# Intsights/PySubstringSearch

Hardware: AMD Instinct MI355X
Metric: queries/sec (batched) + index-build GB/s on 512MB chunk, 1/2/4/8 GPU (higher is better)
Workload: dtype u64

## Files before the change

pysubstringsearch_amd/csrc/msd_sort.hip:

```cpp
#include "msd_sort.h"

#include <algorithm>
#include <vector>

#include "prims.h"
#include "scan.h"
#include "text_keys.h"

namespace pss {

constexpr int MSD_D = 10;
constexpr u32 MSD_BINS = 1u << MSD_D;
constexpr int MSD_BLOCK = 512;
constexpr int MSD_WAVES = MSD_BLOCK / kWave;
constexpr int MSD_IPT = 16;
constexpr u32 MSD_TILE = MSD_BLOCK * MSD_IPT;
constexpr u32 MSD_WIN = 6144;
#ifndef PSS_LS_WINDOW
#define PSS_LS_WINDOW 8
#endif
constexpr u32 MSD_TILE_CAP = 8184 - PSS_LS_WINDOW;
constexpr u32 MSD_MAX_BUCKET = 4088;
constexpr int MSD_TAG_BITS = MSD_D + 1;
constexpr u32 MSD_TAG_SPAN = 1u << MSD_TAG_BITS;
// ... 682 lines not shown
struct InNonEmpty {
    const u32 *J;
    __device__ u64 operator()(u64 j) const { return J[j + 1] > J[j] ? 1u : 0u; }
};

__global__ __launch_bounds__(256) void msd_compact_kernel(const u32 *J, u32 nb, const u64 *rank, u32 *cstart, u32 *counters, u32 *cj)
{
    u32 mx = 0;
    for (u32 j = blockIdx.x * blockDim.x + threadIdx.x; j < nb; j += gridDim.x * blockDim.x) {
        const u32 s = J[j], e = J[j + 1];
        if (e > s) {
            cstart[rank[j]] = s;
            if (cj) cj[rank[j]] = j;
            mx = max(mx, e - s);
        }
    }
    mx = wave_incl_max(mx);
    if (lane_id() == kWave - 1 && mx) atomicMax(&counters[1], mx);
}

struct TilePlan {
    u32 win, cap;
    const u32 *cj;
};
__device__ __forceinline__ bool msd_tile_head(const u32 *cstart, u32 ne, u32 n, u32 k, TilePlan tp)
{
    if (tp.cj) {
        if (k == 0 || (tp.cj[k] >> MSD_RAW_TAG_BITS) != (tp.cj[k - 1] >> MSD_RAW_TAG_BITS)) return true;
    } else if ((k & (MSD_TAG_SPAN - 1u)) == 0) {
        return true;
    }
    const u32 w = cstart[k] / tp.win;
    if (cstart[k - 1] / tp.win != w) return true;
    if (k + 1 < ne && cstart[k + 1] / tp.win == w) return false;
    u32 lo = 0, hi = k;
    const u32 ws = w * tp.win;
    while (lo < hi) {
        const u32 mid = (lo + hi) >> 1;
        if (cstart[mid] < ws) lo = mid + 1; else hi = mid;
    }
    const u32 end = k + 1 < ne ? cstart[k + 1] : n;
    return end - cstart[lo] > tp.cap;
}

struct InTileHead {
    const u32 *cstart;
    u32 ne, n;
    TilePlan tp;
    __device__ u64 operator()(u64 k) const { return msd_tile_head(cstart, ne, n, (u32)k, tp) ? 1u : 0u; }
};

struct InTileHeadDev {
    const u32 *cstart;
    const u64 *nep;
    u32 n;
    TilePlan tp;
    __device__ u64 operator()(u64 k) const
    {
        const u32 ne = (u32)*nep;
        return (k < ne && msd_tile_head(cstart, ne, n, (u32)k, tp)) ? 1u : 0u;
    }
};
__global__ __launch_bounds__(256) void msd_tiles_dev_kernel(const u32 *cstart, const u64 *nep, u32 n, const u64 *rank, const u64 *total,
                                                              u32 *tile_first, TilePlan tp)
{
    const u32 ne = (u32)*nep;
    if (blockIdx.x == 0 && threadIdx.x == 0) tile_first[*total] = ne;
    for (u32 k = blockIdx.x * blockDim.x + threadIdx.x; k < ne; k += gridDim.x * blockDim.x) {
        if (msd_tile_head(cstart, ne, n, k, tp)) tile_first[rank[k]] = k;
    }
}

__global__ __launch_bounds__(256) void msd_tiles_kernel(const u32 *cstart, u32 ne, u32 n, const u64 *rank, const u64 *total,
                                                          u32 *tile_first, TilePlan tp)
{
    if (blockIdx.x == 0 && threadIdx.x == 0) tile_first[*total] = ne;
    for (u32 k = blockIdx.x * blockDim.x + threadIdx.x; k < ne; k += gridDim.x * blockDim.x) {
        if (msd_tile_head(cstart, ne, n, k, tp)) tile_first[rank[k]] = k;
    }
}

struct MsdTile {
    u32 e0, count, tag0, nb;
};


struct MsdEmit {
    u32 *st_pos, *st_idx;
    u32 *blk_cnt;
};

__device__ __forceinline__ void msd_emit_tile(const u64 *exch, u32 count, u32 e0, int idx_bits, u32 *sa_out, const MsdEmit *em,
                                              u32 *s_count)
{
    const u32 tid = threadIdx.x, lane = tid & 63u;
    const u32 imask = (u32)((1ull << idx_bits) - 1ull);
    const u32 rows = (count + MSD_BLOCK - 1) / MSD_BLOCK;
#pragma unroll 1
    for (u32 r = 0; r < rows; ++r) {
        const u32 p = r * MSD_BLOCK + tid;
        const bool valid = p < count;
        u64 x = 0;
        bool tie = false;
        if (valid) {
            x = exch[p];
            tie = p > 0 && (exch[p - 1] >> idx_bits) == (x >> idx_bits);
            sa_out[e0 + p] = ((u32)x & imask) | ((tie && em == nullptr) ? 0x80000000u : 0u);
        }
        if (em != nullptr) {
            const u64 tm = __ballot(tie);
            const bool tie_next = lane < 63 ? ((tm >> (lane + 1)) & 1ull) != 0
                                            : (p + 1 < count && (exch[p + 1] >> idx_bits) == (x >> idx_bits));
            if (valid && (tie || tie_next)) {
                const u32 slot = e0 + atomicAdd(s_count, 1u);
                em->st_pos[slot] = e0 + p;
                em->st_idx[slot] = ((u32)x & imask) | (tie ? 0x80000000u : 0u);
            }
        }
    }
}

struct InBlkCnt {
    const u32 *c;
    __device__ u64 operator()(u64 t) const { return c[t]; }
};

constexpr u32 GA_WORDS = MSD_TILE / 32;
__global__ __launch_bounds__(256) void msd_gather_kernel(const MsdTile *tiles, const u32 *blk_cnt, const u64 *dst_off, u32 nt,
                                                           const u32 *st_pos, const u32 *st_idx, u32 *pos, u32 *idx, u32 *grp)
{
    __shared__ u32 s_occ[4][GA_WORDS], s_head[4][GA_WORDS], s_pre[4][GA_WORDS];
    const u32 w = wave_id(), lane = lane_id();
    const u32 t = blockIdx.x * 4 + w;
    if (t >= nt) return;
    const u32 c = blk_cnt[t];
    if (c == 0) return;
    const u32 e0 = tiles[t].e0;
    const u64 d = dst_off[t];
    u32 *occ = s_occ[w], *head = s_head[w], *pre = s_pre[w];
    for (u32 i = lane; i < GA_WORDS; i += kWave) occ[i] = head[i] = 0;
    __builtin_amdgcn_fence(__ATOMIC_ACQ_REL, "wavefront");
    __builtin_amdgcn_wave_barrier();
    for (u32 i = lane; i < c; i += kWave) {
        const u32 q = st_pos[e0 + i] - e0;
        atomicOr(&occ[q >> 5], 1u << (q & 31u));
        if (!(st_idx[e0 + i] >> 31)) atomicOr(&head[q >> 5], 1u << (q & 31u));
    }
    __builtin_amdgcn_fence(__ATOMIC_ACQ_REL, "wavefront");
    __builtin_amdgcn_wave_barrier();
    {
        const u32 c0 = __popc(occ[4 * lane]), c1 = __popc(occ[4 * lane + 1]), c2 = __popc(occ[4 * lane + 2]),
                  c3 = __popc(occ[4 * lane + 3]);
        const u32 ex = wave_incl_sum(c0 + c1 + c2 + c3) - (c0 + c1 + c2 + c3);
        pre[4 * lane] = ex;
        pre[4 * lane + 1] = ex + c0;
        pre[4 * lane + 2] = ex + c0 + c1;
        pre[4 * lane + 3] = ex + c0 + c1 + c2;
    }
    __builtin_amdgcn_fence(__ATOMIC_ACQ_REL, "wavefront");
    __builtin_amdgcn_wave_barrier();
    for (u32 i = lane; i < c; i += kWave) {
        const u32 ps = st_pos[e0 + i], q = ps - e0;
        const u32 below = (q & 31u) ? (occ[q >> 5] & ((1u << (q & 31u)) - 1u)) : 0u;
        const u32 rank = pre[q >> 5] + __popc(below);
        u32 wi = q >> 5;
        u32 m = head[wi] & ((q & 31u) == 31u ? ~0u : ((2u << (q & 31u)) - 1u));
        while (m == 0 && wi > 0) m = head[--wi];
        const u32 hq = wi * 32 + (31u - (u32)__builtin_clz(m | 1u));
        pos[d + rank] = ps;
        idx[d + rank] = st_idx[e0 + i] & 0x7fffffffu;
        grp[d + rank] = e0 + hq + 1;
    }
}


__global__ __launch_bounds__(MSD_BLOCK) void msd_local_sort_kernel(const u64 *in, const MsdTile *tiles, int rem_bits, int idx_bits,
                                                                     u32 *sa_out, const u32 *tile_list, int fused, MsdEmit em_val)
{
    const MsdEmit *em = fused ? &em_val : nullptr;
    __shared__ __attribute__((aligned(16))) u64 exch[MSD_TILE];
    __shared__ u32 wave_hist[MSD_WAVES][256];
    __shared__ u32 scr[MSD_WAVES + 1];
    const u32 tid = threadIdx.x, lane = tid & 63u, wave = tid >> 6;
    const u32 t = tile_list ? tile_list[blockIdx.x] : blockIdx.x;
    const MsdTile td = tiles[t];
    const u32 e0 = td.e0, count = td.count;
    for (u32 i = tid; i < MSD_WAVES * 256; i += MSD_BLOCK) (&wave_hist[0][0])[i] = 0;
    __syncthreads();
    int seg_bits = 0;
    while ((1u << seg_bits) < td.nb) ++seg_bits;
    const u64 tag_base = (u64)td.tag0 << (rem_bits + idx_bits);
    u64 key[MSD_IPT];
#pragma unroll
    for (int r = 0; r < MSD_IPT; ++r) {
        const u32 p = wave * (kWave * MSD_IPT) + r * kWave + lane;
        key[r] = p < count ? in[e0 + p] - tag_base : ~0ull;
    }
    const int sort_bits = rem_bits + seg_bits;
    for (int shift = idx_bits; shift < idx_bits + sort_bits; shift += 8) {
        const int left = idx_bits + sort_bits - shift;
        const u32 dmask = left >= 8 ? 0xffu : ((1u << left) - 1u);
        u32 rank[MSD_IPT], prev[MSD_IPT];
#pragma unroll
        for (int r = 0; r < MSD_IPT; ++r) {
            const bool pad = wave * (kWave * MSD_IPT) + r * kWave + lane >= count;
            const u32 d = pad ? dmask : ((u32)(key[r] >> shift) & dmask);
            const u64 peers = match_digit8(d, ~0ull);
            const u32 below = mbcnt(peers);
            prev[r] = 0;
            if (below == 0) prev[r] = atomicAdd(&wave_hist[wave][d], (u32)__popcll(peers));
            rank[r] = below | ((u32)__builtin_ctzll(peers) << 16);
        }
#pragma unroll
        for (int r = 0; r < MSD_IPT; ++r) rank[r] = __shfl(prev[r], (int)(rank[r] >> 16)) + (rank[r] & 0xffffu);
        __syncthreads();
        {
            u32 c[MSD_WAVES];
            u32 total = 0;
            if (tid < 256) {
#pragma unroll
                for (int w = 0; w < MSD_WAVES; ++w) {
                    c[w] = wave_hist[w][tid];
                    total += c[w];
                }
            }
            const u32 incl = wave_incl_sum(total);
            if (lane == kWave - 1) scr[wave] = incl;
            __syncthreads();
            if (tid < 256) {
                u32 run = incl - total;
                for (u32 w = 0; w < wave; ++w) run += scr[w];
#pragma unroll
                for (int w = 0; w < MSD_WAVES; ++w) {
                    wave_hist[w][tid] = run;
                    run += c[w];
                }
            }
        }
        __syncthreads();
#pragma unroll
        for (int r = 0; r < MSD_IPT; ++r) {
            const bool pad = wave * (kWave * MSD_IPT) + r * kWave + lane >= count;
            const u32 d = pad ? dmask : ((u32)(key[r] >> shift) & dmask);
            exch[wave_hist[wave][d] + rank[r]] = key[r];
        }
        __syncthreads();
        for (u32 i = tid; i < MSD_WAVES * 256; i += MSD_BLOCK) (&wave_hist[0][0])[i] = 0;
#pragma unroll
        for (int r = 0; r < MSD_IPT; ++r) key[r] = exch[wave * (kWave * MSD_IPT) + r * kWave + lane];
        __syncthreads();
    }
    if (sort_bits <= 0) {
#pragma unroll
        for (int r = 0; r < MSD_IPT; ++r) exch[wave * (kWave * MSD_IPT) + r * kWave + lane] = key[r];
        __syncthreads();
    }
    if (tid == 0) scr[0] = 0;
    __syncthreads();
    msd_emit_tile(exch, count, e0, idx_bits, sa_out, em, &scr[0]);
    __syncthreads();
    if (em && tid == 0) em->blk_cnt[t] = scr[0];
}


#ifndef PSS_LS_BIN_BITS
#define PSS_LS_BIN_BITS 12
#endif
constexpr int LS_BIN_BITS = PSS_LS_BIN_BITS;
constexpr u32 LS_BINS = 1u << LS_BIN_BITS;
constexpr u32 LS_WORDS = LS_BINS / 2;
constexpr u32 LS_KMAX = 64;
#ifndef PSS_LS_GROUP
#define PSS_LS_GROUP 1
#endif
constexpr int LS_GROUP = PSS_LS_GROUP;
constexpr int LS_WINDOW = PSS_LS_WINDOW;

__global__ __launch_bounds__(256) void msd_tile_desc_kernel(const u32 *cstart, const u32 *tile_first, u32 nt, u32 ne, u32 n,
                                                              MsdTile *tiles, const u32 *cj, const u64 *ntp, const u64 *nep)
{
    const u32 t = blockIdx.x * blockDim.x + threadIdx.x;
    if (ntp) {
        nt = (u32)*ntp;
        ne = (u32)*nep;
    }
    if (t >= nt) return;
    const u32 k0 = tile_first[t], k1 = tile_first[t + 1];
    const u32 e0 = cstart[k0], e1 = k1 < ne ? cstart[k1] : n;
    if (cj) {
        const u32 t0 = cj[k0] & (MSD_RAW_TAG_SPAN - 1u), t1 = cj[k1 - 1] & (MSD_RAW_TAG_SPAN - 1u);
        tiles[t] = MsdTile{e0, e1 - e0, t0, t1 - t0 + 1u};
    } else {
        tiles[t] = MsdTile{e0, e1 - e0, k0 & (MSD_TAG_SPAN - 1u), k1 - k0};
    }
}

__device__ __forceinline__ void keep_load(u64 &v) { asm volatile("" : "+v"(v)); }

__device__ __forceinline__ void lds_barrier()
{
    asm volatile("s_waitcnt lgkmcnt(0)\n\ts_barrier" ::: "memory");
}

__global__ __launch_bounds__(MSD_BLOCK, 4) void msd_local_fast_kernel(const u64 *in, const MsdTile *tiles, u32 nt, int rem_bits,
                                                                     int idx_bits, u32 *sa_out, u32 *fail_list, u32 *fail_count,
                                                                     int fused, MsdEmit em_val, const u64 *nt_dev,
                                                                     const u32 *counters_dev, const u32 *bad_dev)
{
    if (nt_dev) {
        if (counters_dev[1] > MSD_MAX_BUCKET || (bad_dev && *bad_dev)) return;
        nt = (u32)*nt_dev;
    }
    const MsdEmit *em = fused ? &em_val : nullptr;
    __shared__ __attribute__((aligned(16))) u64 lds_all[MSD_TILE + LS_WORDS];
    u64 *const exch = lds_all;
    u32 *const hist = reinterpret_cast<u32 *>(lds_all + MSD_TILE);
    u32 *const hist2 = hist + LS_WORDS;
    u32 *const scr = reinterpret_cast<u32 *>(&exch[MSD_TILE - 8]);
    u32 &s_fail = scr[MSD_WAVES + 2];
    const u32 tid = threadIdx.x;
    const u32 stride = gridDim.x;
    u32 t = blockIdx.x;
    if (t >= nt) return;
    MsdTile cur = tiles[t];
    MsdTile nxt = t + stride < nt ? tiles[t + stride] : MsdTile{0, 0, 0, 0};
    u64 pe[MSD_IPT];
    auto prefetch = [&](const MsdTile &d) {
#pragma unroll
        for (int r = 0; r < MSD_IPT; ++r) {
            const u32 p = r * MSD_BLOCK + tid;
            pe[r] = p < d.count ? in[d.e0 + p] : 0ull;
        }
    };
    prefetch(cur);
    for (u32 i = tid; i < LS_WORDS; i += MSD_BLOCK) hist[i] = 0;
    if (tid == 0) {
        s_fail = 0;
        scr[MSD_WAVES + 3] = 0;
    }
    lds_barrier();
    u32 prev_t = 0;
    bool prev_ok = false;
    for (;;) {
        const u32 count = cur.count, e0 = cur.e0;
        const u32 rows = (count + MSD_BLOCK - 1) / MSD_BLOCK;
        int seg_bits = 0;
        while ((1u << seg_bits) < cur.nb) ++seg_bits;
        const u64 tag_base = (u64)cur.tag0 << (rem_bits + idx_bits);
        const int sort_bits = rem_bits + seg_bits;
        const int bin_shift = idx_bits + (sort_bits > LS_BIN_BITS ? sort_bits - LS_BIN_BITS : 0);
        u64 e[MSD_IPT];
#pragma unroll
        for (int r = 0; r < MSD_IPT; ++r) {
            e[r] = ~0ull;
            if ((u32)r < rows) {
                const u32 p = r * MSD_BLOCK + tid;
                if (p < count) {
                    e[r] = pe[r] - tag_base;
                    const u32 bin = (u32)(e[r] >> bin_shift);
                    atomicAdd(&hist[bin >> 1], 1u << (16u * (bin & 1u)));
                }
            }
        }
        const bool more = t + stride < nt;
        if (more) prefetch(nxt);
        lds_barrier();
        if (tid == 0) {
            if (em && prev_ok) em->blk_cnt[prev_t] = scr[MSD_WAVES + 3];
            s_fail = 0;
            scr[MSD_WAVES + 3] = 0;
        }
        {
            constexpr int LS_WPT = LS_WORDS / MSD_BLOCK;
            static_assert(LS_WPT * MSD_BLOCK == (int)LS_WORDS && LS_WPT >= 1, "bins split evenly over the threads");
            u32 c[2 * LS_WPT];
            u32 sum = 0;
#pragma unroll
            for (int j = 0; j < LS_WPT; ++j) {
                const u32 wv = hist[LS_WPT * tid + j];
                c[2 * j] = wv & 0xffffu;
                c[2 * j + 1] = wv >> 16;
                sum += c[2 * j] + c[2 * j + 1];
            }
            const u32 incl = wave_incl_sum(sum);
            if (lane_id() == kWave - 1) scr[wave_id()] = incl;
            lds_barrier();
            u32 ex = incl - sum;
            for (int w = 0; w < wave_id(); ++w) ex += scr[w];
#pragma unroll
            for (int j = 0; j < LS_WPT; ++j) {
                const u32 lo = ex, hi = ex + c[2 * j];
                hist[LS_WPT * tid + j] = hist2[LS_WPT * tid + j] = lo | (hi << 16);
                ex = hi + c[2 * j + 1];
            }
        }
        lds_barrier();
#pragma unroll
        for (int r = 0; r < MSD_IPT; ++r) {
            if ((u32)r < rows) {
                const u32 p = r * MSD_BLOCK + tid;
                if (p < count) {
                    const u32 bin = (u32)(e[r] >> bin_shift), sh = 16u * (bin & 1u);
                    exch[(atomicAdd(&hist2[bin >> 1], 1u << sh) >> sh) & 0xffffu] = e[r];
                }
            }
        }
        if (tid < (u32)LS_WINDOW) exch[count + tid] = ~0ull;
        lds_barrier();
        const u16 *const starts16 = reinterpret_cast<const u16 *>(hist);
        u32 rk[MSD_IPT];
#pragma unroll
        for (int g = 0; g < MSD_IPT; g += LS_GROUP) {
            if ((u32)g < rows) {
                u64 x[LS_GROUP];
                u32 s0[LS_GROUP], sm[LS_GROUP];
#pragma unroll
                for (int j = 0; j < LS_GROUP; ++j) x[j] = exch[(g + j) * MSD_BLOCK + tid];
#pragma unroll
                for (int j = 0; j < LS_GROUP; ++j) {
                    const u32 bin = (u32)(x[j] >> bin_shift) & (LS_BINS - 1u);
                    s0[j] = starts16[bin];
                }
                u64 y[LS_GROUP][LS_WINDOW];
#pragma unroll
                for (int j = 0; j < LS_GROUP; ++j) {
#pragma unroll
                    for (int k = 0; k < LS_WINDOW; ++k) y[j][k] = exch[s0[j] + k];
                }
#pragma unroll
                for (int j = 0; j < LS_GROUP; ++j) {
                    u32 c = 0;
#pragma unroll
                    for (int k = 0; k < LS_WINDOW; ++k) {
                        keep_load(y[j][k]);
                        c += y[j][k] < x[j] ? 1u : 0u;
                    }
                    sm[j] = c;
                }
#pragma unroll
                for (int j = 0; j < LS_GROUP; ++j) {
                    const u32 p = (g + j) * MSD_BLOCK + tid;
                    if (p < count && ((y[j][LS_WINDOW - 1] ^ x[j]) >> bin_shift) == 0) {
                        const u32 bin = (u32)(x[j] >> bin_shift) & (LS_BINS - 1u);
                        const u32 s1 = bin + 1u < LS_BINS ? (u32)starts16[min(bin + 1u, LS_BINS - 1u)] : count;
                        const u32 len = s1 - s0[j];
                        if (len > LS_KMAX) {
                            s_fail = 1;
                        } else {
                            for (u32 q = s0[j] + LS_WINDOW; q < s0[j] + len; ++q) sm[j] += exch[q] < x[j] ? 1u : 0u;
                        }
                    }
                    e[g + j] = x[j];
                    rk[g + j] = s0[j] + sm[j];
                }
            } else {
#pragma unroll
                for (int j = 0; j < LS_GROUP; ++j) rk[g + j] = 0;
            }
        }
        lds_barrier();
        const bool failed = s_fail != 0;
        if (failed) {
            if (tid == 0) fail_list[atomicAdd(fail_count, 1u)] = t;
        } else {
#pragma unroll
            for (int r = 0; r < MSD_IPT; ++r) {
                if ((u32)r < rows) {
                    const u32 p = r * MSD_BLOCK + tid;
                    if (p < count) exch[rk[r]] = e[r];
                }
            }
        }
        for (u32 i = tid; i < LS_WORDS; i += MSD_BLOCK) hist[i] = 0;
        lds_barrier();
        if (!failed) {
            const u32 imask = (u32)((1ull << idx_bits) - 1ull);
            u32 *const s_count = &scr[MSD_WAVES + 3];
#pragma unroll
            for (int g = 0; g < MSD_IPT; g += LS_GROUP) {
                if ((u32)g < rows) {
                    u64 cur[LS_GROUP], prv[LS_GROUP], nxt[LS_GROUP];
#pragma unroll
                    for (int j = 0; j < LS_GROUP; ++j) {
                        const u32 p = (g + j) * MSD_BLOCK + tid;
                        cur[j] = exch[p];
                        prv[j] = exch[p ? p - 1 : 0];
                        nxt[j] = exch[p + 1];
                    }
#pragma unroll
                    for (int j = 0; j < LS_GROUP; ++j) {
                        keep_load(cur[j]);
                        keep_load(prv[j]);
                        keep_load(nxt[j]);
                    }
#pragma unroll
                    for (int j = 0; j < LS_GROUP; ++j) {
                        const u32 p = (g + j) * MSD_BLOCK + tid;
                        if (p < count) {
                            const u64 kx = cur[j] >> idx_bits;
                            const bool tie = p > 0 && (prv[j] >> idx_bits) == kx;
                            const u32 sfx = (u32)cur[j] & imask;
                            sa_out[e0 + p] = sfx | ((tie && em == nullptr) ? 0x80000000u : 0u);
                            if (em != nullptr) {
                                const bool tie_next = p + 1 < count && (nxt[j] >> idx_bits) == kx;
                                if (tie || tie_next) {
                                    const u32 slot = e0 + atomicAdd(s_count, 1u);
                                    em->st_pos[slot] = e0 + p;
                                    em->st_idx[slot] = sfx | (tie ? 0x80000000u : 0u);
                                }
                            }
                        }
                    }
                }
            }
        }
        prev_t = t;
        prev_ok = !failed;
        if (!more) break;
        t += stride;
        cur = nxt;
        nxt = t + stride < nt ? tiles[t + stride] : MsdTile{0, 0, 0, 0};
    }
    if (em) {
        lds_barrier();
        if (tid == 0 && prev_ok) em->blk_cnt[prev_t] = scr[MSD_WAVES + 3];
    }
}

#include "ss_sort_impl.h"


static size_t msd_max_tiles(uint32_t n)
{
    return (size_t)n / (SS_WIN / 2) + ((size_t)MSD_BINS * MSD_BINS) / MSD_RAW_TAG_SPAN + 8;
}

static size_t msd_max_tiles2(uint32_t n) { return (size_t)n / MSD_TILE2 + MSD_BINS + 8; }

static bool msd_use_lsd(uint32_t n)
{
    const char *e = knob("PSS_MSD_LSD");
    return !(e && atoi(e) == 0) && n < (1u << 30);
}

size_t msd_workspace_bytes(uint32_t n)
{
    const size_t max_ranges2 = (size_t)n / MSD_G2_RANGE + MSD_BINS + 8;
    const size_t nbk = (size_t)MSD_BINS * MSD_BINS;
    return max_ranges2 * MSD_BINS * 4
           + (MSD_BINS + 8) * 4
           + (nbk + 8) * 4
           + max_ranges2 * sizeof(MsdRange) + (MSD_BINS + 8) * 4 + 64
           + (nbk + 8) * 8
           + (nbk + 8) * 4
           + (msd_max_tiles(n) + 32) * 8
           + (msd_max_tiles(n) + 32) * 16
           + (msd_max_tiles(n) + 32) * sizeof(MsdTile)
           + (SC_MAX_BLOCKS + 8) * 8 + 8192
           + (size_t)MSD_BINS * MSD_G1_RANGES * 4 + (MSD_BINS + 8) * 4
           + msd_max_tiles2(n) * (sizeof(MsdTile2) + (size_t)MSD_BINS * 4)
           + (nbk + 8) * 4 + 4096;
}

int msd_max_key_bits(uint32_t n)
{
    int ib = 1;
    while ((1ull << ib) < (u64)n) ++ib;
    const int after2 = 64 + MSD_D - (msd_use_lsd(n) ? MSD_RAW_TAG_BITS : MSD_TAG_BITS) - ib + MSD_D;
    return std::min(after2, 64 + MSD_D - ib);
}

int msd_suffix_sort(DeviceCtx *ctx, const TextKeys *text, uint32_t n, int key_bits, uint64_t *A[2], uint32_t *sa_out,
                    void *work, uint32_t *h_small, bool profile, MsdStats *stats, bool *accepted, MsdActive *active,
                    const MsdFront *front)
{
    *accepted = false;
    hipStream_t s = ctx->stream;
    int ib = 1;
    while ((1ull << ib) < (u64)n) ++ib;
    if (key_bits < 2 * MSD_D + 1 || key_bits > msd_max_key_bits(n) || n < 2) {
        set_error("msd_suffix_sort: key of %d bits does not fit (n = %u)", key_bits, n);
        return PSS_EINVAL;
    }
    const size_t max_ranges2 = (size_t)n / MSD_G2_RANGE + MSD_BINS + 8;
    const size_t nbk = (size_t)MSD_BINS * MSD_BINS;
    u8 *w = static_cast<u8 *>(work);
    size_t o = 0;
    auto carve = [&](size_t bytes) { u8 *p = w + o; o = round_up(o + bytes, 256); return p; };
    u32 *T = reinterpret_cast<u32 *>(carve(max_ranges2 * MSD_BINS * 4));
    u32 *J1 = reinterpret_cast<u32 *>(carve((MSD_BINS + 8) * 4));
    u32 *J = reinterpret_cast<u32 *>(carve((nbk + 8) * 4));
    MsdRange *ranges2 = reinterpret_cast<MsdRange *>(carve(max_ranges2 * sizeof(MsdRange)));
    u32 *seg_first = reinterpret_cast<u32 *>(carve((MSD_BINS + 8) * 4));
    u32 *counters = reinterpret_cast<u32 *>(carve(64));
    u64 *ranks = reinterpret_cast<u64 *>(carve((nbk + 8) * 8));
    u32 *cstart = reinterpret_cast<u32 *>(carve((nbk + 8) * 4));
    const size_t max_tiles = msd_max_tiles(n);
    MsdTile *tiles_all = reinterpret_cast<MsdTile *>(carve((max_tiles + 16) * sizeof(MsdTile)));
    u32 *tile_first = reinterpret_cast<u32 *>(carve((max_tiles + 16) * 8));
    u32 *blk_cnt = reinterpret_cast<u32 *>(carve((max_tiles + 8) * 4));
    u64 *dst_off = reinterpret_cast<u64 *>(carve((max_tiles + 8) * 8));
    u64 *partial = reinterpret_cast<u64 *>(carve((SC_MAX_BLOCKS + 8) * 8));
    u64 *d_total = partial + SC_MAX_BLOCKS;
    const bool lsd = msd_use_lsd(n);
    const size_t max_tiles2 = msd_max_tiles2(n);
    u32 *T2 = nullptr, *Jb = nullptr, *status = nullptr, *cj = nullptr;
    MsdTile2 *tiles2 = nullptr;
    if (lsd) {
        T2 = reinterpret_cast<u32 *>(carve((size_t)MSD_BINS * MSD_G1_RANGES * 4));
        Jb = reinterpret_cast<u32 *>(carve((MSD_BINS + 8) * 4));
        tiles2 = reinterpret_cast<MsdTile2 *>(carve(max_tiles2 * sizeof(MsdTile2)));
        status = reinterpret_cast<u32 *>(carve(max_tiles2 * MSD_BINS * 4));
        cj = reinterpret_cast<u32 *>(carve((nbk + 8) * 4));
    }

    MsdArgs a;
    memset(&a, 0, sizeof a);
    a.codes = text->codes;
    a.code_bits = text->code_bits;
    a.key_chars = text->key_chars;
    a.plus_one = text->plus_one;
    a.key_drop = text->drop;
    a.n = n;
    a.key_bits = key_bits;
    a.idx_bits = ib;
    const u32 num_tiles = (u32)(((u64)n + MSD_TILE - 1) / MSD_TILE);
    a.tiles_per_range1 = (num_tiles + MSD_G1_RANGES - 1) / MSD_G1_RANGES;
    a.num_ranges1 = (num_tiles + a.tiles_per_range1 - 1) / a.tiles_per_range1;
    a.T = T;
    a.J1 = J1;
    a.J = J;
    a.ranges2 = ranges2;
    a.seg_first = seg_first;
    a.counters = counters;
    a.lsd = lsd ? 1 : 0;
    a.T2 = T2;
    a.Jb = Jb;
    a.tiles2 = tiles2;
    a.status = status;

    hipEvent_t ev[8] = {};
    int nev = 0;
    struct EvGuard {
        hipEvent_t *e;
        int *n;
        ~EvGuard()
        {
            for (int i = 0; i < *n; ++i) (void)hipEventDestroy(e[i]);
        }
    } guard{ev, &nev};
    auto mark = [&]() -> int {
        if (profile && nev < 8) {
            PSS_HIP(hipEventCreate(&ev[nev]));
            PSS_HIP(hipEventRecord(ev[nev], s));
            ++nev;
        }
        return PSS_OK;
    };

    PSS_HIP(hipMemsetAsync(counters, 0, 64, s));
    a.out = A[0];
    if (front) {
        a.raw = front->raw;
        a.lut = front->lut;
        a.codes_out = const_cast<u8 *>(text->codes);
        a.bad = front->bad;
        hipLaunchKernelGGL(msd_hist_raw_kernel, dim3(a.num_ranges1), dim3(MSD_BLOCK), 0, s, a);
    } else {
        hipLaunchKernelGGL(msd_hist_kernel<true>, dim3(a.num_ranges1), dim3(MSD_BLOCK), 0, s, a);
    }
    static_assert(MSD_G1_RANGES <= 1024, "msd_offsets1_kernel takes four ranges per thread");
    hipLaunchKernelGGL(msd_offsets1_kernel, dim3(MSD_BINS), dim3(256), 0, s, T, a.num_ranges1, seg_first);
    hipLaunchKernelGGL(msd_offsets1b_kernel, dim3(1), dim3(MSD_BINS), 0, s, (const u32 *)seg_first, J1, n);
    if (lsd) {
        hipLaunchKernelGGL(msd_offsets1_kernel, dim3(MSD_BINS), dim3(256), 0, s, T2, a.num_ranges1, seg_first);
        hipLaunchKernelGGL(msd_offsets1b_kernel, dim3(1), dim3(MSD_BINS), 0, s, (const u32 *)seg_first, Jb, n);
        PSS_HIP(hipMemsetAsync(status, 0, max_tiles2 * MSD_BINS * 4, s));
    }
    PSS_TRY(mark());
    const bool wide = lsd || !(knob("PSS_MSD_SCATTER") && atoi(knob("PSS_MSD_SCATTER")) == 1);
    if (lsd) hipLaunchKernelGGL((msd_scatter2_kernel<true, 1024, true>), dim3(a.num_ranges1), dim3(1024), 0, s, a);
    else if (wide) hipLaunchKernelGGL((msd_scatter2_kernel<true, 1024>), dim3(a.num_ranges1), dim3(1024), 0, s, a);
    else hipLaunchKernelGGL(msd_scatter_kernel<true>, dim3(a.num_ranges1), dim3(MSD_BLOCK), 0, s, a);
    PSS_TRY(mark());
    a.in = A[0];
    a.out = A[1];
    if (lsd) {
        hipLaunchKernelGGL(msd_tiles2_kernel, dim3(1), dim3(MSD_BINS), 0, s, (const u32 *)J1, tiles2, counters);
        PSS_TRY(mark());
        const u32 grid2 = std::min<u32>((u32)max_tiles2, (u32)ctx->num_cus);
        hipLaunchKernelGGL(msd_scatter_lb_kernel, dim3(grid2), dim3(1024), 0, s, a);
        PSS_TRY(mark());
    } else {
        hipLaunchKernelGGL(msd_ranges_kernel, dim3(1), dim3(MSD_BINS), 0, s, J1, ranges2, seg_first, counters);
        a.dense = ranks;
        hipLaunchKernelGGL(msd_hist_kernel<false>, dim3((u32)max_ranges2), dim3(MSD_BLOCK), 0, s, a);
        hipLaunchKernelGGL(msd_offsets_kernel, dim3(MSD_BINS), dim3(MSD_BINS), 0, s, T, (const u32 *)seg_first, (const u32 *)J1, J,
                           0u, n, MSD_BINS);
    }
    PSS_TRY(device_excl_scan(ctx, InNonEmpty{J}, nbk, partial, d_total, ranks));
    hipLaunchKernelGGL(msd_compact_kernel, dim3(1024), dim3(256), 0, s, J, (u32)nbk, ranks, cstart, counters, cj);
    const int rem_bits = key_bits - 2 * MSD_D;
    MsdEmit em{};
    const int fused = active != nullptr;
    if (fused) em = MsdEmit{active->st_pos, active->st_idx, blk_cnt};
    const bool one_trip = lsd && !knob("PSS_MSD_SLOW_LOCAL");
    u64 *d_total2 = d_total + 1;
    u32 *const fail_list_dev = tile_first + max_tiles + 16;
    if (one_trip) {
        const TilePlan tpd{MSD_WIN, MSD_TILE_CAP, cj};
        PSS_TRY(device_excl_scan(ctx, InTileHeadDev{cstart, d_total, n, tpd}, nbk, partial, d_total2, ranks));
        hipLaunchKernelGGL(msd_tiles_dev_kernel, dim3(1024), dim3(256), 0, s, cstart, (const u64 *)d_total, n, ranks, (const u64 *)d_total2,
                           tile_first, tpd);
        hipLaunchKernelGGL(msd_tile_desc_kernel, dim3((u32)((max_tiles + 255) / 256)), dim3(256), 0, s, cstart, tile_first, 0u, 0u, n,
                           tiles_all, (const u32 *)cj, (const u64 *)d_total2, (const u64 *)d_total);
        PSS_TRY(mark());
        hipLaunchKernelGGL(msd_local_fast_kernel, dim3(2u * (u32)ctx->num_cus), dim3(MSD_BLOCK), 0, s, A[1], (const MsdTile *)tiles_all, 0u,
                           rem_bits, ib, sa_out, fail_list_dev, counters + 4, fused, em, (const u64 *)d_total2, (const u32 *)counters,
                           front ? (const u32 *)front->bad : (const u32 *)nullptr);
        PSS_TRY(mark());
        PSS_HIP(hipMemcpyAsync(h_small + 8, d_total2, 8, hipMemcpyDeviceToHost, s));
        PSS_HIP(hipMemcpyAsync(h_small + 10, counters + 4, 4, hipMemcpyDeviceToHost, s));
    }
    PSS_HIP(hipMemcpyAsync(h_small, d_total, 8, hipMemcpyDeviceToHost, s));
    PSS_HIP(hipMemcpyAsync(h_small + 2, counters, 16, hipMemcpyDeviceToHost, s));
    if (front) PSS_HIP(hipMemcpyAsync(h_small + 6, front->bad, 4, hipMemcpyDeviceToHost, s));
    PSS_HIP(hipStreamSynchronize(s));
    const u32 ne = h_small[0];
    const u32 maxb = h_small[3];
    if (stats) {
        stats->buckets = ne;
        stats->max_bucket = maxb;
        stats->bad_symbol = front ? h_small[6] : 0u;
    }
    if (front && h_small[6]) return PSS_OK;
    if (maxb > MSD_MAX_BUCKET) return PSS_OK;
    if (!lsd) {
        PSS_TRY(mark());
        if (wide) hipLaunchKernelGGL((msd_scatter2_kernel<false, 1024>), dim3((u32)max_ranges2), dim3(1024), 0, s, a);
        else hipLaunchKernelGGL(msd_scatter_kernel<false>, dim3((u32)max_ranges2), dim3(MSD_BLOCK), 0, s, a);
        PSS_TRY(mark());
    }
    const auto local_sort = msd_local_sort_kernel;
    const auto local_fast = msd_local_fast_kernel;
    u32 nt = 0;
    u32 *fail_list = fail_list_dev;
    if (one_trip) {
        nt = h_small[8];
        if ((size_t)nt > max_tiles) {
            set_error("msd_suffix_sort: %u tiles planned, tables hold %zu (internal error)", nt, max_tiles);
            return PSS_EDEVICE;
        }
        const u32 nfail = h_small[10];
        if (stats) stats->slow_tiles = nfail;
        if (nfail)
            hipLaunchKernelGGL(local_sort, dim3(nfail), dim3(MSD_BLOCK), 0, s, A[1], (const MsdTile *)tiles_all, rem_bits,
                               ib, sa_out, (const u32 *)fail_list, fused, em);
    } else {
    const TilePlan tp{MSD_WIN, MSD_TILE_CAP, cj};
    PSS_TRY(device_excl_scan(ctx, InTileHead{cstart, ne, n, tp}, ne, partial, d_total, ranks));
    hipLaunchKernelGGL(msd_tiles_kernel, dim3(1024), dim3(256), 0, s, cstart, ne, n, ranks, (const u64 *)d_total, tile_first, tp);
    PSS_HIP(hipMemcpyAsync(h_small, d_total, 8, hipMemcpyDeviceToHost, s));
    PSS_HIP(hipStreamSynchronize(s));
    nt = h_small[0];
    if ((size_t)nt > max_tiles) {
        set_error("msd_suffix_sort: %u tiles planned, tables hold %zu (internal error)", nt, max_tiles);
        return PSS_EDEVICE;
    }
    PSS_TRY(mark());
    fail_list = tile_first + nt + 8;
    hipLaunchKernelGGL(msd_tile_desc_kernel, dim3((nt + 255) / 256), dim3(256), 0, s, cstart, tile_first, nt, ne, n, tiles_all,
                       (const u32 *)cj, (const u64 *)nullptr, (const u64 *)nullptr);
    if (knob("PSS_MSD_SLOW_LOCAL")) {
        hipLaunchKernelGGL(local_sort, dim3(nt), dim3(MSD_BLOCK), 0, s, A[1], (const MsdTile *)tiles_all, rem_bits, ib,
                           sa_out, (const u32 *)nullptr, fused, em);
    } else {
        MsdTile *tiles = tiles_all;
        const u32 grid = std::min<u32>(nt, 2u * (u32)ctx->num_cus);
        hipLaunchKernelGGL(local_fast, dim3(grid), dim3(MSD_BLOCK), 0, s, A[1], (const MsdTile *)tiles, nt, rem_bits, ib,
                           sa_out, fail_list, counters + 4, fused, em, (const u64 *)nullptr, (const u32 *)nullptr, (const u32 *)nullptr);
        PSS_TRY(mark());
        PSS_HIP(hipMemcpyAsync(h_small, counters + 4, 4, hipMemcpyDeviceToHost, s));
        PSS_HIP(hipStreamSynchronize(s));
        const u32 nfail = h_small[0];
        if (stats) stats->slow_tiles = nfail;
        if (nfail)
            hipLaunchKernelGGL(local_sort, dim3(nfail), dim3(MSD_BLOCK), 0, s, A[1], (const MsdTile *)tiles_all, rem_bits,
                               ib, sa_out, (const u32 *)fail_list, fused, em);
    }
    if (knob("PSS_MSD_SLOW_LOCAL")) PSS_TRY(mark());
    }
    if (fused) {
        PSS_TRY(device_excl_scan(ctx, InBlkCnt{blk_cnt}, nt, partial, d_total, dst_off));
        hipLaunchKernelGGL(msd_gather_kernel, dim3((nt + 3) / 4), dim3(256), 0, s, (const MsdTile *)tiles_all, blk_cnt, dst_off, nt,
                           active->st_pos, active->st_idx, active->pos, active->idx, active->grp);
        PSS_HIP(hipMemcpyAsync(h_small, d_total, 8, hipMemcpyDeviceToHost, s));
        PSS_HIP(hipStreamSynchronize(s));
        active->count = h_small[0];
    }
    PSS_HIP(hipGetLastError());
    if (stats) {
        stats->tiles = nt;
        stats->lookback = lsd ? 1u : 0u;
    }
    if (profile && nev >= 6) {
        PSS_HIP(hipStreamSynchronize(s));
        float ms = 0.f;
        PSS_HIP(hipEventElapsedTime(&ms, ev[0], ev[1]));
        if (stats) stats->ms_g1 = ms;
        PSS_HIP(hipEventElapsedTime(&ms, ev[2], ev[3]));
        if (stats) stats->ms_g2 = ms;
        PSS_HIP(hipEventElapsedTime(&ms, ev[4], ev[5]));
        if (stats) stats->ms_local = ms;
// ... 283 lines not shown
```

Baseline: 67.07.

## Use buffer loads/stores with range-clamped descriptors and wave-ballot tie detection in local sort

Tile prefetch loads and the suffix-array output stores now go through raw buffer instructions whose resource descriptor is sized to the tile's remaining elements. Out-of-range lanes are masked by the hardware instead of per-element compare branches. The tie-detection epilogue drops the neighbour load of the next element: it reads only the current and previous entries and derives the 'tie with next' flag from a wave ballot shifted by one lane, plus a precomputed cross-row edge mask. Tile fields are made wave-uniform with readfirstlane, and the seg_bits loop is replaced with clz. This relies on the tie semantics exactly matching the old per-element checks at wave and row boundaries.

```diff
diff --git a/pysubstringsearch_amd/csrc/msd_sort.hip b/pysubstringsearch_amd/csrc/msd_sort.hip
--- a/pysubstringsearch_amd/csrc/msd_sort.hip
+++ b/pysubstringsearch_amd/csrc/msd_sort.hip
@@ -1008,6 +1008,13 @@
     asm volatile("s_waitcnt lgkmcnt(0)\n\ts_barrier" ::: "memory");
 }
 
+__device__ __forceinline__ u32 uniform(u32 v) { return (u32)__builtin_amdgcn_readfirstlane((int)v); }
+
+__device__ __forceinline__ __amdgpu_buffer_rsrc_t tile_rsrc(const void *base, u32 bytes)
+{
+    return __builtin_amdgcn_make_buffer_rsrc(const_cast<void *>(base), (short)0, (int)bytes, 0x00020000);
+}
+
 __global__ __launch_bounds__(MSD_BLOCK, 4) void msd_local_fast_kernel(const u64 *in, const MsdTile *tiles, u32 nt, int rem_bits,
                                                                      int idx_bits, u32 *sa_out, u32 *fail_list, u32 *fail_count,
                                                                      int fused, MsdEmit em_val, const u64 *nt_dev,
@@ -1031,14 +1038,17 @@
     MsdTile cur = tiles[t];
     MsdTile nxt = t + stride < nt ? tiles[t + stride] : MsdTile{0, 0, 0, 0};
     u64 pe[MSD_IPT];
-    auto prefetch = [&](const MsdTile &d) {
+    const u32 voff8 = tid * 8u, voff4 = tid * 4u;
+    auto prefetch = [&](u32 pe0, u32 pcount) {
 #pragma unroll
         for (int r = 0; r < MSD_IPT; ++r) {
-            const u32 p = r * MSD_BLOCK + tid;
-            pe[r] = p < d.count ? in[d.e0 + p] : 0ull;
+            const u32 first = r * MSD_BLOCK;
+            const u32 left = uniform(max(pcount, first) - first);
+            const auto v = __builtin_amdgcn_raw_buffer_load_b64(tile_rsrc(in + pe0 + first, left * 8u), (int)voff8, 0, 0);
+            pe[r] = (u64)v[0] | ((u64)v[1] << 32);
         }
     };
-    prefetch(cur);
+    prefetch(uniform(cur.e0), uniform(cur.count));
     for (u32 i = tid; i < LS_WORDS; i += MSD_BLOCK) hist[i] = 0;
     if (tid == 0) {
         s_fail = 0;
@@ -1048,17 +1058,16 @@
     u32 prev_t = 0;
     bool prev_ok = false;
     for (;;) {
-        const u32 count = cur.count, e0 = cur.e0;
+        const u32 count = uniform(cur.count), e0 = uniform(cur.e0), nb = uniform(cur.nb);
         const u32 rows = (count + MSD_BLOCK - 1) / MSD_BLOCK;
-        int seg_bits = 0;
-        while ((1u << seg_bits) < cur.nb) ++seg_bits;
-        const u64 tag_base = (u64)cur.tag0 << (rem_bits + idx_bits);
+        const int seg_bits = nb > 1u ? 32 - __builtin_clz(nb - 1u) : 0;
+        const u64 tag_base = (u64)uniform(cur.tag0) << (rem_bits + idx_bits);
         const int sort_bits = rem_bits + seg_bits;
         const int bin_shift = idx_bits + (sort_bits > LS_BIN_BITS ? sort_bits - LS_BIN_BITS : 0);
         u64 e[MSD_IPT];
 #pragma unroll
         for (int r = 0; r < MSD_IPT; ++r) {
-            e[r] = ~0ull;
+            e[r] = 0;
             if ((u32)r < rows) {
                 const u32 p = r * MSD_BLOCK + tid;
                 if (p < count) {
@@ -1069,7 +1078,7 @@
             }
         }
         const bool more = t + stride < nt;
-        if (more) prefetch(nxt);
+        if (more) prefetch(uniform(nxt.e0), uniform(nxt.count));
         lds_barrier();
         if (tid == 0) {
             if (em && prev_ok) em->blk_cnt[prev_t] = scr[MSD_WAVES + 3];
@@ -1180,41 +1189,39 @@
         for (u32 i = tid; i < LS_WORDS; i += MSD_BLOCK) hist[i] = 0;
         lds_barrier();
         if (!failed) {
-            const u32 imask = (u32)((1ull << idx_bits) - 1ull);
+            const u64 tie_lim = 1ull << idx_bits;
+            const u32 imask = (u32)(tie_lim - 1ull);
+            const u32 flag = em == nullptr ? 0x80000000u : 0u;
+            const u32 lane = tid & (kWave - 1u);
+            u32 edge = 0;
+            if (em != nullptr) {
+                const u32 q = lane * MSD_BLOCK + (tid - lane) + kWave;
+                bool te = false;
+                if (lane < (u32)MSD_IPT && q < count) te = (exch[q] ^ exch[q - 1]) < tie_lim;
+                edge = (u32)__builtin_amdgcn_ballot_w64(te);
+            }
             u32 *const s_count = &scr[MSD_WAVES + 3];
-#pragma unroll
-            for (int g = 0; g < MSD_IPT; g += LS_GROUP) {
-                if ((u32)g < rows) {
-                    u64 cur[LS_GROUP], prv[LS_GROUP], nxt[LS_GROUP];
-#pragma unroll
-                    for (int j = 0; j < LS_GROUP; ++j) {
-                        const u32 p = (g + j) * MSD_BLOCK + tid;
-                        cur[j] = exch[p];
-                        prv[j] = exch[p ? p - 1 : 0];
-                        nxt[j] = exch[p + 1];
-                    }
-#pragma unroll
-                    for (int j = 0; j < LS_GROUP; ++j) {
-                        keep_load(cur[j]);
-                        keep_load(prv[j]);
-                        keep_load(nxt[j]);
-                    }
-#pragma unroll
-                    for (int j = 0; j < LS_GROUP; ++j) {
-                        const u32 p = (g + j) * MSD_BLOCK + tid;
-                        if (p < count) {
-                            const u64 kx = cur[j] >> idx_bits;
-                            const bool tie = p > 0 && (prv[j] >> idx_bits) == kx;
-                            const u32 sfx = (u32)cur[j] & imask;
-                            sa_out[e0 + p] = sfx | ((tie && em == nullptr) ? 0x80000000u : 0u);
-                            if (em != nullptr) {
-                                const bool tie_next = p + 1 < count && (nxt[j] >> idx_bits) == kx;
-                                if (tie || tie_next) {
-                                    const u32 slot = e0 + atomicAdd(s_count, 1u);
-                                    em->st_pos[slot] = e0 + p;
-                                    em->st_idx[slot] = sfx | (tie ? 0x80000000u : 0u);
-                                }
-                            }
+            const u32 rec_bytes = em != nullptr ? count * 4u : 0u;
+            const auto r_pos = tile_rsrc(em != nullptr ? em->st_pos + e0 : sa_out, rec_bytes);
+            const auto r_idx = tile_rsrc(em != nullptr ? em->st_idx + e0 : sa_out, rec_bytes);
+            const u32 pv0 = tid ? tid - 1u : 0u;
+#pragma unroll
+            for (int r = 0; r < MSD_IPT; ++r) {
+                if ((u32)r < rows) {
+                    const u32 first = r * MSD_BLOCK, left = count - first;
+                    const u64 c = exch[first + tid];
+                    const u64 pv = exch[r ? first + tid - 1u : pv0];
+                    const bool tie = ((c ^ pv) < tie_lim) && tid < left && (r > 0 || tid > 0);
+                    const u32 sfx = (u32)c & imask;
+                    __builtin_amdgcn_raw_buffer_store_b32(sfx | (tie ? flag : 0u), tile_rsrc(sa_out + e0 + first, left * 4u),
+                                                          (int)voff4, 0, 0);
+                    if (em != nullptr) {
+                        const u64 tm = __builtin_amdgcn_ballot_w64(tie);
+                        const u64 rec = tm | (tm >> 1) | ((u64)((edge >> r) & 1u) << (kWave - 1));
+                        if (__builtin_amdgcn_inverse_ballot_w64(rec)) {
+                            const u32 slot = atomicAdd(s_count, 1u) * 4u;
+                            __builtin_amdgcn_raw_buffer_store_b32(e0 + first + tid, r_pos, (int)slot, 0, 0);
+                            __builtin_amdgcn_raw_buffer_store_b32(sfx | (tie ? 0x80000000u : 0u), r_idx, (int)slot, 0, 0);
                         }
                     }
                 }
```

Measured after the change: 65.93. 1.7% lower.
